# alexncoleman/WeaklySupervisedDL

Measured on AMD Instinct MI355X. Metric: SegmentationModel train img/s at B=16 256x256, higher is better.
Workload: dtype f32

## Files before the change

### include/wsdl_hip.h

```cpp
#ifndef WSDL_HIP_H
#define WSDL_HIP_H

#include <stddef.h>
#include <stdint.h>

#ifdef __cplusplus
extern "C" {
#endif

typedef void* wsdl_stream_t;

enum {
    WSDL_OK = 0,
    WSDL_EINVAL = -1,
    WSDL_EHIP = -2,
    WSDL_EWORKSPACE = -3
};

const char* wsdl_last_error(void);
int wsdl_launch_trace(int on);
const char* wsdl_last_launches(void);
int wsdl_version(void);
const char* wsdl_target_arch(void);

int wsdl_set_option(const char* name, int value);

enum { WSDL_PROF_IGEMM_128x128_A = 0,
       WSDL_PROF_IGEMM_128x128_U = 1,
       WSDL_PROF_IGEMM_128x64_A = 2, WSDL_PROF_IGEMM_128x64_U = 3,
       WSDL_PROF_IGEMM_64x256_A = 4, WSDL_PROF_IGEMM_64x256_U = 5,
       WSDL_PROF_IGEMM_64x128_A = 6, WSDL_PROF_IGEMM_64x128_U = 7,
       WSDL_PROF_WGRAD_128x128 = 8,
       WSDL_PROF_WGRAD_64x128 = 9,
       WSDL_PROF_WGRAD_FAST_128x128 = 10,
       WSDL_PROF_PAIRWISE = 11, WSDL_PROF_LAYERCAM = 12,
       WSDL_PROF_SPLIT_128x128 = 13,
       WSDL_PROF_SPLIT_128x64 = 14, WSDL_PROF_SPLIT_64x256 = 15, WSDL_PROF_SPLIT_64x128 = 16,
       WSDL_PROF_WGRAD_SPLIT32 = 17,
       WSDL_PROF_SPLIT_256x128 = 18,
       WSDL_PROF_STEM = 19,
       WSDL_PROF_WGRAD_SPLIT16D = 20,
       WSDL_PROF_SPLIT_GROUP = 21,
       WSDL_PROF_SPLIT_MULTI = 22,
       WSDL_PROF_NCLASSES = 23 };
const char* wsdl_prof_class_name(int cls);
int wsdl_prof_enable(int on);
int wsdl_prof_collect(int cls, long long* launches, double* total_ms, double* total_work,
                      double* total_work_executed ,
                      double* total_bytes );
int wsdl_prof_reset(void);

int wsdl_range_enable(int on);
int wsdl_range_push(const char* name);
int wsdl_range_pop(void);


size_t wsdl_conv2d_weight_layout_bytes(int Cout, int Cin, int kh, int kw, int dgrad, int* is_plain);
int wsdl_conv2d_prep_weights(const float* w, void* wt_fwd, void* wt_dgrad,
                             int Cout, int Cin, int kh, int kw,
                             const float* w_amax ,
                             wsdl_stream_t stream);

int wsdl_conv2d_fwd(const float* x, const void* wt_fwd, float* y,
                    int B, int Cin, int H, int W, int Cout, int kh, int kw,
                    int stride, int pad, int dil,
                    const float* scale, const float* shift, const float* residual, int relu,
                    long long x_bs, long long y_bs, long long res_bs,
                    const float* x_amax ,
                    float* y_amax ,
                    void* ws, size_t ws_bytes, wsdl_stream_t stream);
typedef struct wsdl_prep_desc {
    const float* w;
    void* wt_fwd;
    void* wt_dgrad;
    const float* w_amax;
    int Cout, Cin, taps, grid_x;
    int block_begin, reserved;
} wsdl_prep_desc;
int wsdl_conv2d_prep_weights_multi(const wsdl_prep_desc* desc, int n, int total_blocks, wsdl_stream_t stream);

size_t wsdl_conv2d_igemm_workspace(int B, int Cin, int H, int W, int Cout, int kh, int kw,
                                   int stride, int pad, int dil, int dgrad);

int wsdl_conv2d_dgrad(const float* dy, const void* wt_dgrad, float* dx,
                      int B, int Cin, int H, int W, int Cout, int kh, int kw,
                      int stride, int pad, int dil, int accumulate, const uint8_t* acc_mask,
                      long long dy_bs, const float* dy_amax, void* ws, size_t ws_bytes, wsdl_stream_t stream);
int wsdl_conv2d_fwd_group_ok(int n, int B, int Cin, int H, int W, int Cout);
size_t wsdl_conv2d_fwd_group_workspace(int n, const int* k, const int* dil, int B, int Cin, int H, int W, int Cout);
int wsdl_conv2d_fwd_group(int n, const float* x, const void* const* wt_fwd, float* const* y, const int* k, const int* dil,
                          int B, int Cin, int H, int W, int Cout, long long x_bs, const long long* y_bs,
                          const float* x_amax, void* ws, size_t ws_bytes, wsdl_stream_t stream);
int wsdl_conv2d_dgrad_multi_ok(int n, int B, int Cin, int H, int W, int Cout);
int wsdl_conv2d_dgrad_multi(int n, const float* const* dy, const void* const* wt_dgrad, const float* const* dy_amax,
                            const int* k, const int* dil, const long long* dy_bs, float* dx, int B, int Cin, int H, int W,
                            int Cout, int accumulate, wsdl_stream_t stream);

// ... 218 lines not shown
```

### weaklysuperviseddl_amd/csrc/common.hip

```cpp
#include "common.h"

#include <dlfcn.h>

#include <algorithm>
#include <mutex>
#include <vector>

namespace wsdl {

static thread_local char g_err[512] = "";
Opt g_range_sentinel{0};

void set_error(const char* fmt, ...) {
    va_list ap;
    va_start(ap, fmt);
    vsnprintf(g_err, sizeof(g_err), fmt, ap);
    va_end(ap);
}

std::atomic<int> g_trace_launches{0};
static thread_local char g_trace[2048] = "";
static thread_local size_t g_trace_len = 0;
void trace_launch(const char* fmt, ...) {
    if (g_trace_len + 4 >= sizeof(g_trace)) return;
// ... 47 lines not shown
    } else {
        if (hipEventCreate(&r.start) != hipSuccess) return;
        if (hipEventCreate(&r.stop) != hipSuccess) return;
    }
    (void)hipEventRecord(r.start, s);
    g_prof[cls].push_back(r);
    slot = reinterpret_cast<void*>(g_prof[cls].size());
}

ProfScope::~ProfScope() {
    if (g_ranges_on) g_roctx_pop();
    if (!slot) return;
    std::lock_guard<std::mutex> lk(g_prof_mu);
    size_t idx = reinterpret_cast<size_t>(slot) - 1;
    if (idx < g_prof[cls].size()) (void)hipEventRecord(g_prof[cls][idx].stop, s);
}

}

extern "C" {

int wsdl_launch_trace(int on) {
    wsdl::g_trace_launches.store(on ? 1 : 0);
    wsdl::g_trace[0] = 0;
    wsdl::g_trace_len = 0;
    return WSDL_OK;
}

const char* wsdl_last_launches(void) {
    static thread_local char out[sizeof(wsdl::g_trace)];
    memcpy(out, wsdl::g_trace, sizeof(out));
    wsdl::g_trace[0] = 0;
    wsdl::g_trace_len = 0;
    return out;
}

const char* wsdl_last_error(void) { return wsdl::g_err; }
int wsdl_version(void) { return 200; }
const char* wsdl_target_arch(void) { return "gfx950"; }

const char* wsdl_prof_class_name(int cls) {
    static const char* names[WSDL_PROF_NCLASSES] = {
        "conv_igemm_fast_kernel<128, 128, 2, 16>", "conv_igemm_kernel<128, 128, 2, false>",
        "conv_igemm_fast_kernel<128, 64, 2, 32>", "conv_igemm_kernel<128, 64, 2, false>",
        "conv_igemm_fast_kernel<64, 256, 1, 16>", "conv_igemm_kernel<64, 256, 1, false>",
        "conv_igemm_fast_kernel<64, 128, 1, 32>", "conv_igemm_kernel<64, 128, 1, false>",
        "conv_wgrad_kernel<128, 128, 2>", "conv_wgrad_kernel<64, 128, 1>", "conv_wgrad_fast_kernel<128, 128, 2, 16>",
        "pairwise_kernel", "layercam_partial_kernel",
        "conv_igemm_split_kernel<128, 128, 2, 16, 256, AR>", "conv_igemm_split_kernel<128, 64, 2, 32, 256, AR>",
        "conv_igemm_split_kernel<64, 256, 1, 16, 256, AR>", "conv_igemm_split_kernel<64, 128, 1, 32, 256, AR>",
        "conv_wgrad_split16_kernel<128, 128, false>", "conv_igemm_split_kernel<256, 128, 4, BK, 512, AR, false, false>",
        "stem_conv7x7s2_kernel", "conv_wgrad_split16d_kernel<MODE, DYRAW>",
        "conv_igemm_split_group_kernel<256, 128, 4, 16, 512, AR, false>",
        "conv_igemm_split_kernel<256, 128, 4, 16, 512, AR, false, true>"};
    return cls >= 0 && cls < WSDL_PROF_NCLASSES ? names[cls] : "?";
}

int wsdl_range_enable(int on) {
    if (on && !wsdl::load_roctx()) {
        wsdl::set_error("range_enable: librocprofiler-sdk-roctx.so / libroctx64.so could not be loaded");
        return WSDL_EINVAL;
    }
    wsdl::g_ranges_on = on != 0;
    return WSDL_OK;
}
int wsdl_range_push(const char* name) {
    if (wsdl::g_ranges_on && name) wsdl::g_roctx_push(name);
    return WSDL_OK;
}
int wsdl_range_pop(void) {
    if (wsdl::g_ranges_on) wsdl::g_roctx_pop();
    return WSDL_OK;
}

int wsdl_prof_enable(int on) {
    std::lock_guard<std::mutex> lk(wsdl::g_prof_mu);
    wsdl::g_prof_on = on != 0;
    return WSDL_OK;
}

int wsdl_prof_reset(void) {
    std::lock_guard<std::mutex> lk(wsdl::g_prof_mu);
    for (auto& v : wsdl::g_prof) {
        for (auto& r : v) wsdl::g_free_events.emplace_back(r.start, r.stop);
        v.clear();
    }
    return WSDL_OK;
}

int wsdl_prof_collect(int cls, long long* launches, double* total_ms, double* total_work,
                      double* total_work_executed, double* total_bytes) {
    WSDL_REQUIRE(cls >= 0 && cls < WSDL_PROF_NCLASSES, "prof class %d out of range", cls);
    std::lock_guard<std::mutex> lk(wsdl::g_prof_mu);
    double ms = 0.0, work = 0.0, exe = 0.0, byt = 0.0;
    for (auto& r : wsdl::g_prof[cls]) {
        WSDL_HIP_CHECK(hipEventSynchronize(r.stop));
        float t = 0.f;
        WSDL_HIP_CHECK(hipEventElapsedTime(&t, r.start, r.stop));
        ms += t;
        work += r.work;
        exe += r.executed;
        byt += r.bytes;
    }
    if (launches) *launches = (long long)wsdl::g_prof[cls].size();
    if (total_ms) *total_ms = ms;
    if (total_work) *total_work = work;
    if (total_work_executed) *total_work_executed = exe;
// ... 6 lines not shown
```

### weaklysuperviseddl_amd/csrc/conv_igemm.hip

```cpp
#include "common.h"

#include <type_traits>
#include <algorithm>
#include <cstdint>
#include <mutex>

typedef float f32x16 __attribute__((ext_vector_type(16)));

namespace {

constexpr int kThreads = 256;

struct ConvSrc {
    const float* x;
    const float* wt;
    const float* x_amax;
    int KH, KW, bh, ch, K, Cin;
    long long x_bs;
    unsigned x_bytes;
};

struct ConvP {
    const float* x;
    const float* wt;
// ... 1602 lines not shown
    bool fast;
    wgrad_tile(Cout, Cin, &BM, &BN, &fast);
    long long tiles = (long long)wsdl::cdiv(Cout, BM) * wsdl::cdiv(N, BN);
    const int chunks = wsdl::cdiv(P, 32);
    const long long smax = std::max<long long>(1, std::min<long long>(256, chunks / 8));
    if (wgrad_chunk32(Cout, Cin, N)) {
        tiles = (long long)wsdl::cdiv(Cout, BM) * wsdl::cdiv(std::max(n_live, BN), BN);
        const long long slots = 2 * kNumCU;
        long long best_s = 1;
        double best = -1.0;
        for (long long c = 1; c <= smax && tiles * c <= 5 * slots / 2; ++c) {
            const long long blocks = tiles * c, rounds = (blocks + slots - 1) / slots;
            double eff = (double)blocks / (double)(rounds * slots);
            if (blocks < slots) eff *= 0.9;
            if (eff > best + 0.03) { best = eff; best_s = c; }
        }
        if (tap_balance < 0.7 && n_live > BN && best_s + 1 <= smax) ++best_s;
        return (int)best_s;
    }
    long long s0 = (g_wgrad_blocks + tiles - 1) / tiles;
    if (s0 > smax) s0 = smax;
    if (s0 < 1) s0 = 1;
    long long s = s0;
    double best = 0.0;
    for (long long c = std::max<long long>(1, s0 - 1); c <= std::min<long long>(smax, s0 + 3); ++c) {
        const long long blocks = tiles * c, rounds = (blocks + kNumCU - 1) / kNumCU;
        const double eff = (double)blocks / (double)(rounds * kNumCU);
        if (eff > best + 0.02) { best = eff; s = c; }
    }
    return (int)s;
}


__global__ void transpose_add_kernel(const float* __restrict__ t, float* __restrict__ dw, int Cout, int Cin,
                                     int accumulate) {
    __shared__ float tile[32][33];
    const int co0 = blockIdx.x * 32, ci0 = blockIdx.y * 32;
    for (int r = threadIdx.y; r < 32; r += 8) {
        const int ci = ci0 + r, co = co0 + threadIdx.x;
        tile[r][threadIdx.x] = (ci < Cin && co < Cout) ? t[(long long)ci * Cout + co] : 0.f;
    }
    __syncthreads();
    for (int r = threadIdx.y; r < 32; r += 8) {
        const int co = co0 + r, ci = ci0 + threadIdx.x;
        if (co < Cout && ci < Cin) {
            const long long o = (long long)co * Cin + ci;
            dw[o] = accumulate ? dw[o] + tile[threadIdx.x][r] : tile[threadIdx.x][r];
        }
    }
}

bool wgrad_role_swap(int Cin, int Cout, int kh, int kw, int stride, int pad) {
    return kh == 1 && kw == 1 && stride == 1 && pad == 0 && !wgrad_chunk32(Cout, Cin, Cin) && wgrad_chunk32(Cin, Cout, Cout);
}

enum { WGRAD_REDUCE_PLAIN = 0, WGRAD_REDUCE_TILED, WGRAD_REDUCE_VEC4, WGRAD_REDUCE_MANY, WGRAD_REDUCE_MANY16 };
struct WgradReduce {
    const float* slab;
    float* dw;
    unsigned long long live;
    int S, Cout, Cin, T;
    int accumulate, kind;
    int grid_x, nblocks;
};
int wgrad_reduce_one(const WgradReduce& d, hipStream_t s) {
    switch (d.kind) {
        case WGRAD_REDUCE_TILED:
            hipLaunchKernelGGL(wgrad_reduce_tiled_kernel, dim3(d.grid_x, d.Cout), dim3(256), 0, s, d.slab, d.dw, d.S, d.Cout, d.Cin, d.T,
                               d.accumulate, d.live);
            break;
        case WGRAD_REDUCE_VEC4:
            hipLaunchKernelGGL(wgrad_reduce_vec4_kernel, dim3(d.nblocks), dim3(256), 0, s, reinterpret_cast<const float4*>(d.slab),
                               reinterpret_cast<float4*>(d.dw), d.S, (long long)d.Cout * d.Cin * d.T / 4, d.accumulate);
            break;
        case WGRAD_REDUCE_MANY:
            hipLaunchKernelGGL(wgrad_reduce_many_kernel, dim3(d.nblocks), dim3(256), 0, s, d.slab, d.dw, d.S, d.Cout, d.Cin, d.T,
                               d.accumulate, d.live);
            break;
        case WGRAD_REDUCE_MANY16:
            hipLaunchKernelGGL(wgrad_reduce_many16_kernel, dim3(d.nblocks), dim3(256), 0, s, d.slab, d.dw, d.S, d.Cout, d.Cin, d.T,
                               d.accumulate, d.live);
            break;
        default:
            hipLaunchKernelGGL(wgrad_reduce_kernel, dim3(d.nblocks), dim3(256), 0, s, d.slab, d.dw, d.S, d.Cout, d.Cin, d.T, d.accumulate,
                               d.live);
            break;
    }
    WSDL_LAUNCH_CHECK();
    return WSDL_OK;
}

template <int BM, int BN, int WM>
int launch_wgrad_fast(const WgradP& p, hipStream_t s, int S) {
    dim3 grid(p.N / BN, p.Cout / BM, S);
    hipLaunchKernelGGL((conv_wgrad_fast_kernel<BM, BN, WM, 16>), grid, dim3(kThreads), 2 * (BM + BN) * 17 * sizeof(float), s, p);
    WSDL_LAUNCH_CHECK();
    return WSDL_OK;
}

}

extern "C" {

int wsdl_set_option(const char* name, int value) {
    WSDL_REQUIRE(name, "set_option: null name");
    static std::mutex mu;
// ... 494 lines not shown
static int stem_wgrad_grid(int B, int OH, int OW) {
    const long long tiles = (long long)B * wsdl::cdiv(OH, kSwTH) * wsdl::cdiv(OW, kStemTW);
    return (int)std::min<long long>(tiles, kSwMaxGrid);
}

static size_t wgrad_dys_bytes(int Cout, int Cin, int N, int P) {
    if (!wgrad_chunk32(Cout, Cin, N)) return 0;
    const size_t n = (size_t)wsdl::cdiv(P, 32) * Cout * w2row_bytes(g_conv_arith);
    return n < (1ull << 31) ? n : 0;
}

static int wgrad_bands(int Cout, int Cin, int OW, int W, int kw, int stride, int pad, int dil, Band* bands) {
    int BM, BN;
    bool fast;
    wgrad_tile(Cout, Cin, &BM, &BN, &fast);
    bands[0] = Band{0, OW};
    if (!fast || stride != 1) return 1;
    if (wgrad_chunk32(Cout, Cin, kw * kw * Cin)) return 1;
    return column_bands(OW, W, 1, dil, -pad, 1, kw, bands);
}

size_t wsdl_conv2d_wgrad_presplit_bytes(int B, int Cin, int H, int W, int Cout, int kh, int kw, int stride, int pad, int dil) {
    int OH, OW;
    if (check_geom(B, Cin, H, W, Cout, kh, kw, stride, pad, dil, &OH, &OW)) return 0;
    if (g_conv_arith != 1 && g_conv_arith != 2) return 0;
    if (wgrad_role_swap(Cin, Cout, kh, kw, stride, pad)) return 0;
    const int N = kh * kw * Cin, P = B * OH * OW;
    const size_t bytes = wgrad_dys_bytes(Cout, Cin, N, P);
    if (!bytes || P % 32 != 0) return 0;
    const long long xb = (long long)B * Cin * H * W * 4, dyb = (long long)B * Cout * OH * OW * 4;
    if (xb >= (1ll << 31) || dyb >= (1ll << 31)) return 0;
    bool taps_aligned = true;
    for (int kx = 0; kx < kw; ++kx) taps_aligned = taps_aligned && (((kx * dil - pad) & 3) == 0);
    const bool direct = g_wgrad_direct && taps_aligned && stride == 1 && OW % 32 == 0 && W % 4 == 0 && (H * W) % 4 == 0;
    const bool dyraw = direct && g_wgrad_dyraw && (N / 128 <= 10 || g_wgrad_dyraw == 2) && (OH * OW) % 4 == 0;
    return dyraw ? 0 : bytes;
}

size_t wsdl_conv2d_wgrad_workspace(int B, int Cin, int H, int W, int Cout, int kh, int kw, int stride,
                                   int pad, int dil) {
    int OH, OW;
    if (check_geom(B, Cin, H, W, Cout, kh, kw, stride, pad, dil, &OH, &OW)) return 0;
    if (wgrad_role_swap(Cin, Cout, kh, kw, stride, pad))
        return wsdl::align_up((size_t)Cout * Cin * sizeof(float), 256) +
               wsdl_conv2d_wgrad_workspace(B, Cout, OH, OW, Cin, 1, 1, 1, 0, 1);
    const int N = kh * kw * Cin;
    Band bands[8];
    const int nb = wgrad_bands(Cout, Cin, OW, W, kw, stride, pad, dil, bands);
    const int n_live = __builtin_popcountll(live_taps(H, W, OH, OW, kh, kw, stride, pad, dil)) * Cin;
    size_t slabs = (size_t)nb * wgrad_splits(Cout, Cin, N, B * OH * OW, n_live, wgrad_tap_balance(H, OH, kh, stride, pad, dil)) *
                   Cout * N * sizeof(float);
    if (stem_wgrad_eligible(B, Cin, H, W, Cout, kh, kw, stride, pad, dil))
        slabs = std::max(slabs, (size_t)stem_wgrad_grid(B, OH, OW) * Cout * N * sizeof(float));
    return wsdl::align_up(slabs, 256) + wsdl::align_up(wgrad_dys_bytes(Cout, Cin, N, B * OH * OW), 256) +
           (g_wgrad_chan_scale ? wsdl::align_up((size_t)(Cin + Cout) * sizeof(float), 256) : 0);
}

struct WgradExtra {
    const float* x_chan;
    const float* dy_chan;
    const void* dy_presplit;
};
static int wgrad_impl(const float* x, const float* dy, float* dw, int B, int Cin, int H, int W,
                      int Cout, int kh, int kw, int stride, int pad, int dil, int accumulate,
                      long long x_bs, long long dy_bs, const float* x_amax, const float* dy_amax, void* ws,
                      size_t ws_bytes, wsdl_stream_t stream, WgradExtra ex = WgradExtra{}) {
    WSDL_REQUIRE(x && dy && dw && ws, "conv2d_wgrad: null pointer");
    int OH, OW;
    if (int rc = check_geom(B, Cin, H, W, Cout, kh, kw, stride, pad, dil, &OH, &OW)) return rc;
    if (wgrad_role_swap(Cin, Cout, kh, kw, stride, pad)) {
        const size_t t_bytes = wsdl::align_up((size_t)Cout * Cin * sizeof(float), 256);
        WSDL_REQUIRE(ws_bytes > t_bytes, "conv2d_wgrad: workspace too small");
        float* dwt = static_cast<float*>(ws);
        if (int rc = wgrad_impl(dy, x, dwt, B, Cout, OH, OW, Cin, 1, 1, 1, 0, 1, 0,
                                dy_bs ? dy_bs : (long long)Cout * OH * OW, x_bs ? x_bs : (long long)Cin * H * W,
                                dy_amax, x_amax, static_cast<char*>(ws) + t_bytes, ws_bytes - t_bytes, stream,
                                WgradExtra{ex.dy_chan, ex.x_chan, nullptr}))
            return rc;
        WSDL_TRACE("role-swapped (dW^T) + transpose");
        hipLaunchKernelGGL(transpose_add_kernel, dim3(wsdl::cdiv(Cout, 32), wsdl::cdiv(Cin, 32)), dim3(32, 8), 0,
                           wsdl::as_stream(stream), dwt, dw, Cout, Cin, accumulate);
        WSDL_LAUNCH_CHECK();
        return WSDL_OK;
    }
    WgradP p{};
    p.x = x; p.dy = dy; p.slab = static_cast<float*>(ws);
    p.B = B; p.Cin = Cin; p.H = H; p.W = W; p.Cout = Cout; p.OH = OH; p.OW = OW; p.KH = kh; p.KW = kw;
    p.stride = stride; p.pad = pad; p.dil = dil;
    p.N = kh * kw * Cin; p.P = B * OH * OW;
    p.x_bs = x_bs ? x_bs : (long long)Cin * H * W;
    p.dy_bs = dy_bs ? dy_bs : (long long)Cout * OH * OW;
    p.x_amax = x_amax;
    if (stem_wgrad_eligible(B, Cin, H, W, Cout, kh, kw, stride, pad, dil) &&
        (long long)B * wsdl::cdiv(OH, kSwTH) * wsdl::cdiv(OW, kStemTW) < (1ll << 31)) {
        const int G = stem_wgrad_grid(B, OH, OW);
        const size_t need = (size_t)G * Cout * p.N * sizeof(float);
        if (ws_bytes < need) {
            wsdl::set_error("conv2d_wgrad: workspace %zu < %zu bytes", ws_bytes, need);
            return WSDL_EWORKSPACE;
        }
        hipStream_t s = wsdl::as_stream(stream);
        const int tiles_w = wsdl::cdiv(OW, kStemTW), tiles_h = wsdl::cdiv(OH, kSwTH);
        {
            const double flops = 2.0 * p.P * (double)Cout * p.N;
            wsdl::ProfScope prof(WSDL_PROF_WGRAD_64x128, s, flops, flops, 4.0 * ((double)B * Cin * H * W + (double)p.P * Cout + (double)G * Cout * p.N));
            WSDL_TRACE("stem_wgrad7x7s2 fp32 workgroups=%d slabs=%d", G, G);
            hipLaunchKernelGGL(stem_wgrad7x7s2_kernel, dim3(G), dim3(256), 0, s, p, tiles_w, tiles_h, B * tiles_w * tiles_h);
            WSDL_LAUNCH_CHECK();
        }
        WgradReduce rd{};
        rd.slab = p.slab; rd.dw = dw; rd.S = G; rd.Cout = Cout; rd.Cin = Cin; rd.T = kh * kw; rd.accumulate = accumulate;
        rd.live = ~0ull;
        const long long total = (long long)Cout * p.N;
        if (G >= 64) {
            rd.kind = WGRAD_REDUCE_MANY16;
            rd.nblocks = (int)((total + 15) / 16);
        } else if (G >= 16) {
            rd.kind = WGRAD_REDUCE_MANY;
            rd.nblocks = (int)((total + 63) / 64);
        } else {
            rd.kind = WGRAD_REDUCE_PLAIN;
            rd.nblocks = (int)std::min<long long>((total + 255) / 256, 4096);
        }
        WSDL_TRACE("wgrad_reduce slabs=%d", G);
        return wgrad_reduce_one(rd, s);
    }
    const unsigned long long live_all = live_taps(H, W, OH, OW, kh, kw, stride, pad, dil);
    const int S = wgrad_splits(Cout, Cin, p.N, p.P, __builtin_popcountll(live_all) * Cin, wgrad_tap_balance(H, OH, kh, stride, pad, dil));
    Band bands[8];
    const int nb = wgrad_bands(Cout, Cin, OW, W, kw, stride, pad, dil, bands);
    if (nb == 1) bands[0] = Band{0, OW};
    const int S_total = nb * S;
    p.ow0 = 0; p.own = OW; p.slab0 = 0; p.nb = 1; p.splits = S;
    const size_t need = (size_t)S_total * Cout * p.N * sizeof(float);
    if (ws_bytes < need) {
        wsdl::set_error("conv2d_wgrad: workspace %zu < %zu bytes", ws_bytes, need);
        return WSDL_EWORKSPACE;
    }
    const int chunks = wsdl::cdiv(p.P, 32);
    p.chunks_per_split = wsdl::cdiv(chunks, S);
    hipStream_t s = wsdl::as_stream(stream);
    const long long xb = ((long long)(B - 1) * p.x_bs + (long long)Cin * H * W) * 4;
    const long long dyb = ((long long)(B - 1) * p.dy_bs + (long long)Cout * OH * OW) * 4;
    int tBM, tBN;
    bool fast;
    wgrad_tile(Cout, Cin, &tBM, &tBN, &fast);
    if (fast && (xb >= (1ll << 31) || dyb >= (1ll << 31))) {
        const long long img = std::max((long long)Cin * H * W, (long long)Cout * OH * OW) * 4;
        const long long bs = std::max(p.x_bs, p.dy_bs) * 4;
        WSDL_REQUIRE(B > 1 && img < (1ll << 31), "conv2d_wgrad: a single image of 2 GiB or more is not supported");
        long long per = ((1ll << 31) - 4 - img) / bs + 1;
        if (per < 1) per = 1;
        for (int b0 = 0; b0 < B; b0 += (int)per) {
            const int nb_img = (int)std::min<long long>(per, B - b0);
            if (int rc = wgrad_impl(x + (long long)b0 * p.x_bs, dy + (long long)b0 * p.dy_bs, dw, nb_img, Cin, H, W,
                                    Cout, kh, kw, stride, pad, dil, (accumulate || b0 > 0) ? 1 : 0, p.x_bs, p.dy_bs,
                                    x_amax, dy_amax, ws, ws_bytes, stream, WgradExtra{ex.x_chan, ex.dy_chan, nullptr}))
                return rc;
        }
        return WSDL_OK;
    }
    unsigned long long live_mask = ~0ull;
    {
        const double flops = 2.0 * p.P * (double)Cout * p.N;
        double executed = flops;
        const size_t dys_bytes = fast ? wgrad_dys_bytes(Cout, Cin, p.N, p.P) : 0;
        const size_t dys_off = wsdl::align_up(need, 256);
        const bool chunk32 = dys_bytes && ws_bytes >= dys_off + dys_bytes;
        if (wsdl::prof_enabled() && fast) {
            executed = 0.0;
            for (int i = 0; i < nb; ++i)
                executed += flops * ((double)bands[i].own / OW) *
                            wgrad_executed_fraction(B * OH * bands[i].own, OH, bands[i].ow0, bands[i].own, H, W, kh, kw,
                                                    stride, pad, dil, chunk32 ? 32 : 16);
        }
        bool taps_aligned = true;
        for (int kx = 0; kx < kw; ++kx) taps_aligned = taps_aligned && (((kx * dil - pad) & 3) == 0);
        const bool direct = chunk32 && g_conv_arith && g_wgrad_direct && taps_aligned &&
// ... 215 lines not shown
```

### weaklysuperviseddl_amd/csrc/conv_split.h

```cpp
#pragma once

typedef __bf16 bf16x8 __attribute__((ext_vector_type(8)));
typedef __bf16 bf16x2 __attribute__((ext_vector_type(2)));
typedef _Float16 half8 __attribute__((ext_vector_type(8)));
typedef float f32x4 __attribute__((ext_vector_type(4)));

__device__ __forceinline__ void split3(float x0, float x1, unsigned& h, unsigned& m, unsigned& l) {
    f32x2 v = {x0, x1};
    h = __builtin_bit_cast(unsigned, __builtin_convertvector(v, bf16x2));
    f32x2 r = {x0 - __builtin_bit_cast(float, h << 16), x1 - __builtin_bit_cast(float, h & 0xffff0000u)};
    m = __builtin_bit_cast(unsigned, __builtin_convertvector(r, bf16x2));
    f32x2 s = {r[0] - __builtin_bit_cast(float, m << 16), r[1] - __builtin_bit_cast(float, m & 0xffff0000u)};
    l = __builtin_bit_cast(unsigned, __builtin_convertvector(s, bf16x2));
}

__device__ __forceinline__ void split2hs(float x0, float x1, unsigned& h, unsigned& l) {
    f32x2 v = {x0, x1};
    const half2v hv = __builtin_convertvector(v, half2v);
    h = __builtin_bit_cast(unsigned, hv);
    f32x2 r = {(x0 - (float)hv[0]) * 2048.f, (x1 - (float)hv[1]) * 2048.f};
    l = __builtin_bit_cast(unsigned, __builtin_convertvector(r, half2v));
}

template <int AR> struct SplitArith;
// ... 1356 lines not shown
#pragma unroll
            for (int i = 0; i < TMI; ++i) {
                const half8 a0 = *reinterpret_cast<const half8*>(Ab + i * 16 * ROW + fr0);
                const half8 a1 = *reinterpret_cast<const half8*>(Ab + i * 16 * ROW + fr1);
#pragma unroll
                for (int j = 0; j < TNI; ++j) {
                    f32x4 c = acc[i][j];
                    c = __builtin_amdgcn_mfma_f32_16x16x32_f16(a1, b[j][0], c, 0, 0, 0);
                    c = __builtin_amdgcn_mfma_f32_16x16x32_f16(a0, b[j][1], c, 0, 0, 0);
                    c = __builtin_amdgcn_mfma_f32_16x16x32_f16(a0, b[j][0], c, 0, 0, 0);
                    acc[i][j] = c;
                }
            }
            if (c1 < chunk_end) store_a(std::integral_constant<int, 1 - S>{}, buf ^ 1);
            buf ^= 1;
            c0 = c1;
            c1 = c2;
        };
        while (c0 < chunk_end) {
            step(S0{});
            if (c0 >= chunk_end) break;
            step(S1{});
        }
    };
    static_assert(MODE == 0, "only the aligned loop is instantiated (the misaligned-tap loops were removed in round 4)");
    run(std::integral_constant<int, 0>{});

    float* slab = p.slab + (long long)(p.slab0 + bz) * p.Cout * p.N;
    if constexpr (CS) {
#pragma unroll
        for (int i = 0; i < TMI; ++i)
#pragma unroll
            for (int r = 0; r < 4; ++r) {
                const int row = i * 16 + lg * 4 + r, co = m0 + row;
                const int edr = edy_s[row];
#pragma unroll
                for (int j = 0; j < TNI; ++j)
                    slab[(long long)co * p.N + n0 + wid * 32 + j * 16 + l15] = ldexpf(acc[i][j][r], -(exr[j] + edr));
            }
        return;
    }
#pragma unroll
    for (int i = 0; i < TMI; ++i)
#pragma unroll
        for (int j = 0; j < TNI; ++j) {
            const int n = n0 + wid * 32 + j * 16 + l15;
#pragma unroll
            for (int r = 0; r < 4; ++r) {
                const int co = m0 + i * 16 + lg * 4 + r;
                slab[(long long)co * p.N + n] = acc[i][j][r] * out_scale;
            }
        }
}
```

### weaklysuperviseddl_amd/ops.py

```python
import ctypes as C

import os

import threading

import numpy as np
import torch

from ._lib import lib, check, WsdlError

_vp = C.c_void_p


_raw_stream = torch._C._cuda_getCurrentRawStream
_cur_device = torch._C._cuda_getDevice


def raw_stream(device=None):
    idx = device.index if (device is not None and device.index is not None) else _cur_device()
    return _raw_stream(idx)


def _stream():
    return _raw_stream(_cur_device())
# ... 609 lines not shown
    if any(ws[0] != Cout or ws[1] != Cin for ws in wshapes):
        raise WsdlError("conv2d_fwd_group: the problems must share their channel counts")
    IA, PA, LA = C.c_int * n, _vp * n, C.c_longlong * n
    ks, ds = IA(*[int(ws[2]) for ws in wshapes]), IA(*[int(d) for d in dils])
    nws = lib().wsdl_conv2d_fwd_group_workspace(n, ks, ds, B, Cin, H, W, Cout)
    if nws == 0:
        raise WsdlError("conv2d_fwd_group: geometry not supported")
    ws = workspace(nws, x.device)
    if outs is None:
        outs = [torch.empty(B, Cout, H, W, device=x.device, dtype=torch.float32) for _ in range(n)]
    bss = []
    dense = []
    for o in outs:
        t, bs = _planes(o, "out")
        if t is not o:
            raise WsdlError("conv2d_fwd_group: preallocated outputs must be dense planes")
        dense.append(t)
        bss.append(bs)
    check(lib().wsdl_conv2d_fwd_group(n, _p(x), PA(*[_p(w) for w in wfs]), PA(*[_p(t) for t in dense]), ks, ds, B, Cin, H, W,
                                      Cout, x_bs, LA(*bss), _p(x_amax), _p(ws), ws.numel(), _stream()))
    return outs


def dgrad_multi_ok(n, xshape, cout):
    B, Cin, H, W = xshape
    return bool(lib().wsdl_conv2d_dgrad_multi_ok(int(n), B, Cin, H, W, int(cout)))


def conv2d_dgrad_multi(dys, wds, wshapes, dils, xshape, accumulate_into=None, dy_amaxes=None):
    n = len(dys)
    B, Cin, H, W = xshape
    Cout = wshapes[0][0]
    amaxes = []
    dense = []
    bss = []
    for i in range(n):
        if wshapes[i][0] != Cout or wshapes[i][1] != Cin:
            raise WsdlError("conv2d_dgrad_multi: the sources must share their channel counts")
        a = dy_amaxes[i] if dy_amaxes is not None and dy_amaxes[i] is not None else \
            amax_of(dys[i], _split_kc(Cout, wshapes[i][2] * wshapes[i][3]))
        t, bs = _planes(dys[i], "dy")
        amaxes.append(a)
        dense.append(t)
        bss.append(bs)
    dx = accumulate_into if accumulate_into is not None else torch.empty(xshape, device=dys[0].device, dtype=torch.float32)
    PA, IA, LA = _vp * n, C.c_int * n, C.c_longlong * n
    check(lib().wsdl_conv2d_dgrad_multi(n, PA(*[_p(t) for t in dense]), PA(*[_p(w) for w in wds]), PA(*[_p(a) for a in amaxes]),
                                        IA(*[int(ws[2]) for ws in wshapes]), IA(*[int(d) for d in dils]), LA(*bss), _p(dx),
                                        B, Cin, H, W, Cout, int(accumulate_into is not None), _stream()))
    dx._wsdl_fresh = True
    return dx


def _wgrad_split(wshape):
    return CONV_ARITH[0] == 1 and wshape[0] % 128 == 0 and wshape[1] % 128 == 0


def wgrad_presplit_bytes(xshape, wshape, stride, pad, dil):
    B, Cin, H, W = xshape
    Cout, _, kh, kw = wshape
    return _ws_bytes("wsdl_conv2d_wgrad_presplit_bytes", B, Cin, H, W, Cout, kh, kw, stride, pad, dil)


def conv2d_wgrad(x, dy, wshape, stride, pad, dil, out=None, accumulate=False, x_amax=None, dy_amax=None, stream=None,
                 x_camax=None, dy_camax=None, dy_presplit=None):
    if dy_camax is None:
        dy_presplit = None
    elif dy_presplit is None:
        dy_camax_p = getattr(dy, "_wsdl_camax", None)
        if dy_camax_p is dy_camax:
            dy_presplit = getattr(dy, "_wsdl_presplit", None)
    if stream is not None and stream != _stream():
        split = _wgrad_split(wshape)
        if out is None or (split and (x_amax is None or dy_amax is None)):
            raise WsdlError("conv2d_wgrad(stream=): pass out, x_amax and dy_amax (resolved on the current stream)")
        if _planes(x, "x")[0] is not x or _planes(dy, "dy")[0] is not dy:
            raise WsdlError("conv2d_wgrad(stream=): operands must already be dense planes")
    if x_amax is None:
        x_amax = amax_of(x, _wgrad_split(wshape))
    if dy_amax is None:
        dy_amax = amax_of(dy, _wgrad_split(wshape))
    x, x_bs = _planes(x, "x")
    dy, dy_bs = _planes(dy, "dy")
    B, Cin, H, W = x.shape
    Cout, _, kh, kw = wshape
    geom = (B, Cin, H, W, Cout, kh, kw, stride, pad, dil)
    nbytes = _ws_bytes("wsdl_conv2d_wgrad_workspace", *geom)
    if nbytes == 0:
        raise WsdlError("conv2d_wgrad: bad geometry " + repr(geom))
    ws = workspace(nbytes, x.device, stream)
    if out is None:
        out = torch.empty(wshape, device=x.device, dtype=torch.float32)
        accumulate = False
    check(lib().wsdl_conv2d_wgrad_ex(_p(x), _p(dy), _p(out), *geom, int(accumulate), x_bs, dy_bs, _p(x_amax), _p(dy_amax),
                                     _p(x_camax), _p(dy_camax), _p(dy_presplit), _p(ws), ws.numel(),
                                     _stream() if stream is None else stream))
    return out


def bias_grad(dy, out=None, accumulate=False):
    dy, dy_bs = _planes(dy, "dy")
    B, Cc, H, W = dy.shape
    if out is None:
        out = torch.empty(Cc, device=dy.device, dtype=torch.float32)
        accumulate = False
    check(lib().wsdl_bias_grad(_p(dy), _p(out), B, Cc, H * W, dy_bs, int(accumulate), _stream()))
    return out


def bn_fold(bn_weight, bn_bias, running_mean, running_var, eps):
    Cc = bn_weight.numel()
    scale = torch.empty(Cc, device=bn_weight.device, dtype=torch.float32)
    shift = torch.empty_like(scale)
    check(lib().wsdl_bn_fold(_p(_dense(bn_weight)), _p(_dense(bn_bias)), _p(_dense(running_mean)),
                             _p(_dense(running_var)), float(eps), _p(scale), _p(shift), Cc, _stream()))
    return scale, shift


def bn_fold_bias(bn_weight, bn_bias, running_mean, running_var, conv_bias, eps):
    Cc = bn_weight.numel()
    scale = torch.empty(Cc, device=bn_weight.device, dtype=torch.float32)
    shift = torch.empty_like(scale)
    check(lib().wsdl_bn_fold_bias(_p(_dense(bn_weight)), _p(_dense(bn_bias)), _p(_dense(running_mean)),
                                  _p(_dense(running_var)), _p(_dense(conv_bias)), float(eps), _p(scale), _p(shift), Cc,
                                  _stream()))
    return scale, shift


CHAN_AMAX = [os.environ.get("WSDL_CHAN_AMAX", "1") != "0"]
DY_PRESPLIT = [os.environ.get("WSDL_DY_PRESPLIT", "1") != "0"]


def _bn_resident(B, Cc, HW, backward):
    key = ("wsdl_bn_channel_resident", (B, Cc, HW, backward))
# ... 76 lines not shown
    if dx_amax is not None:
        _publish_amax(dx, dx_amax)
    if camax is not None:
        dx._wsdl_camax = camax
        if presplit is not None:
            dx._wsdl_presplit = presplit
    dx._wsdl_fresh = True
    if dres is not None:
        dres._wsdl_fresh = True
    return dx, dgamma, dbeta, dres


def _owned(t):
    return (t is not None and getattr(t, "_wsdl_fresh", False) and t._base is None and t.is_contiguous()
            and t.dtype == torch.float32 and not t.requires_grad)


def affine_act_bwd(dy, y, scale, relu, want_dconv=True, want_dres=False):
    dy = _dense(dy, "dy")
    B, Cc, H, W = dy.shape
    dconv = torch.empty_like(dy) if want_dconv else None
    dres = torch.empty_like(dy) if want_dres else None
    amax = amax_slot(dy.device) if (want_dconv and CONV_ARITH[0] == 1) else None
    check(lib().wsdl_affine_act_bwd(_p(dy), _p(_dense(y) if relu else None), _p(scale), _p(dconv), _p(dres), B, Cc,
                                    H * W, int(relu), _p(amax), _stream()))
    if amax is not None:
        _publish_amax(dconv, amax)
    return dconv, dres


OVERLAP_WGRAD = [True]
WGRAD_AFTER_DGRAD = [False]
LAST_WGRAD_ON_MAIN = [os.environ.get("WSDL_LAST_WGRAD_ON_MAIN", "1") != "0"]
_side_streams = {}


def side_stream(device):
    if device.index is None:
        device = _norm_device(device)
    st = _side_streams.get(device)
    if st is None:
        st = _side_streams[device] = torch.cuda.Stream(device=device)
    return st


def join_side_stream(device):
    st = _side_streams.get(_norm_device(device))
    if st is not None:
        stream_wait(raw_stream(device), st)


def _wgrad_into(param, x, dconv, wshape, stride, pad, dil, sink, x_amax=None, last=False, x_camax=None):
    accumulate = not sink.take_fresh(param)
    split = _wgrad_split(wshape)
    x_amax = x_amax if x_amax is not None else amax_of(x, split)
    dy_amax = amax_of(dconv, split)
    dy_camax = getattr(dconv, "_wsdl_camax", None) if split else None
    dy_presplit = getattr(dconv, "_wsdl_presplit", None) if dy_camax is not None else None
    if not split:
        x_camax = None
    elif x_camax is None:
        x_camax = getattr(x, "_wsdl_camax", None)
    if x_camax is not None and x_camax.numel() != wshape[1]:
        x_camax = None
    if OVERLAP_WGRAD[0] and not (last and LAST_WGRAD_ON_MAIN[0]):
        x, dconv = _planes(x, "x")[0], _planes(dconv, "dy")[0]
        side = side_stream(x.device)
        hside = side.cuda_stream
        stream_wait(hside, _stream())
        conv2d_wgrad(x, dconv, wshape, stride, pad, dil, out=param.grad, accumulate=accumulate, x_amax=x_amax,
                     dy_amax=dy_amax, stream=hside, x_camax=x_camax, dy_camax=dy_camax,
                     dy_presplit=dy_presplit)
        for t in (x_camax, dy_camax, dy_presplit):
            if t is not None:
                t.record_stream(side)
        x.record_stream(side)
        dconv.record_stream(side)
    else:
        conv2d_wgrad(x, dconv, wshape, stride, pad, dil, out=param.grad, accumulate=accumulate, x_amax=x_amax,
                     dy_amax=dy_amax, x_camax=x_camax, dy_camax=dy_camax, dy_presplit=dy_presplit)
    sink.grad_ready(param)


def _sink_of(param):
    sink = getattr(param, "_wsdl_grad_sink", None)
    if sink is None or param.grad is None or not param.grad.is_cuda:
        return None
    return sink


def _alias(t):
    return torch.empty(0, device=t.device, dtype=t.dtype).set_(t.untyped_storage(), t.storage_offset(), t.shape, t.stride())


class IdentityLink:
    __slots__ = ("pending", "projection")

    def __init__(self, projection=False):
        self.pending = None
        self.projection = projection


IDENTITY_LINK = [os.environ.get("WSDL_IDENTITY_LINK", "1") != "0"]


class _ConvBNAct(torch.autograd.Function):

    @staticmethod
    def forward(ctx, x, weight, gamma, beta, residual, running_mean, running_var, stride, pad, dil, relu,
                momentum, eps, cache=None, passthrough=False, link=None, out_holder=None):
        ctx.link = link
        if link is not None:
            ctx.set_materialize_grads(False)
        wf, wd = _cached_prep(cache, weight, x.requires_grad)
        x_amax = amax_of(x, _split_kc(x.shape[1], weight.shape[2] * weight.shape[3]) or _wgrad_split(weight.shape))
        conv = conv2d_fwd(x, wf, weight.shape, stride, pad, dil, x_amax=x_amax)
        y, mean, invstd, rbits = bn_train_fwd(conv, _dense(gamma), _dense(beta), running_mean, running_var, momentum, eps,
                                              residual, relu, out=_alias(out_holder[0]) if out_holder else None,
                                              want_mask=True, mask_if=bool(relu) and residual is not None,
                                              amax_into=out_holder[1] if out_holder else None)
        ctx.cfg = (stride, pad, dil, relu, tuple(weight.shape), tuple(x.shape), residual is not None)
        ctx.params = (weight, gamma, beta)
        ctx.x_amax = x_amax
        ctx.x_camax = getattr(x, "_wsdl_camax", None)
        ctx.save_for_backward(x, conv, y if (relu and residual is not None and rbits is None) else None, gamma, mean, invstd,
                              wd, beta if relu else None, rbits)
        if passthrough:
            xv = x.view_as(x)
            if x_amax is not None:
                _publish_amax(xv, x_amax)
            if ctx.x_camax is not None:
                xv._wsdl_camax = ctx.x_camax
            return y, xv
        return y

    @staticmethod
    def backward(ctx, dy, dxres=None):
        x, conv, y, gamma, mean, invstd, wd, beta_s, rbits = ctx.saved_tensors
        stride, pad, dil, relu, wshape, xshape, has_res = ctx.cfg
        pw, pg, pb = ctx.params
        need_res = has_res and ctx.needs_input_grad[4]
        link = ctx.link
        if dy is None:
            raise WsdlError("conv -> BatchNorm node: no gradient arrived for its output")
        alias_dres = False
        if (link is not None and need_res and rbits is not None and IDENTITY_LINK[0] and tuple(dy.shape) == tuple(conv.shape)
                and dy.is_contiguous()):
            if link.projection:
                link.pending = (dy, rbits)
                need_res, alias_dres = False, True
            elif _owned(dy):
                link.pending = (dy, rbits)
                need_res = False
        shortcut_bits = None
        if link is not None and link.projection and not has_res:
            if link.pending is not None:
                src, shortcut_bits = link.pending
                link.pending = None
                if src.data_ptr() != dy.data_ptr() or tuple(src.shape) != tuple(dy.shape):
                    raise WsdlError("projection shortcut: the gradient that arrived is not the block output's (autograd "
                                    "copied or summed it) - set WSDL_IDENTITY_LINK=0")
        if shortcut_bits is not None:
            relu_b, y_b, beta_b, bits_b = True, None, None, shortcut_bits
        else:
            relu_b, y_b, beta_b, bits_b = relu, y, beta_s, rbits
        sg = _sink_of(pg) if (ctx.needs_input_grad[2] and ctx.needs_input_grad[3] and _sink_of(pg) is _sink_of(pb)) else None
        psb = wgrad_presplit_bytes(xshape, wshape, stride, pad, dil) if (ctx.needs_input_grad[1] and _sink_of(pw) is not None) else 0
        if sg is not None:
# ... 1336 lines not shown


def add_scalars(a, b):
    return _AddAct.apply(a.reshape(1), b.reshape(1), False).reshape(())


def kl_div_batchmean(xn, s):
    return _KLDivBatchMean.apply(xn, s)


RANGES = [False]


def ranges_enable(on=True):
    check(lib().wsdl_range_enable(int(bool(on))))
    RANGES[0] = bool(on)


class prof_range:
    __slots__ = ("name",)

    def __init__(self, name):
        self.name = name

    def __enter__(self):
        if RANGES[0]:
            lib().wsdl_range_push(self.name.encode())

    def __exit__(self, *exc):
        if RANGES[0]:
            lib().wsdl_range_pop()
        return False


if os.environ.get("WSDL_ROCTX") == "1":
    try:
        ranges_enable(True)
    except Exception:
        RANGES[0] = False


PROF_ON = [False]


def prof_enable(on):
    check(lib().wsdl_prof_enable(int(on)))
    PROF_ON[0] = bool(on)


def prof_reset():
    check(lib().wsdl_prof_reset())


PROF_NCLASSES = 23


def prof_class_name(cls):
    return lib().wsdl_prof_class_name(int(cls)).decode()


def prof_collect(cls):
    n, ms, work, exe, byt = C.c_longlong(0), C.c_double(0), C.c_double(0), C.c_double(0), C.c_double(0)
    check(lib().wsdl_prof_collect(int(cls), C.byref(n), C.byref(ms), C.byref(work), C.byref(exe), C.byref(byt)))
    return n.value, ms.value, work.value, exe.value, byt.value
```

Baseline: 916.9.

## Add whole-dW split-fp16 wgrad kernel for small 64-channel convolutions

```diff
diff --git a/include/wsdl_hip.h b/include/wsdl_hip.h
--- a/include/wsdl_hip.h
+++ b/include/wsdl_hip.h
@@ -42,7 +42,8 @@
        WSDL_PROF_WGRAD_SPLIT16D = 20,
        WSDL_PROF_SPLIT_GROUP = 21,
        WSDL_PROF_SPLIT_MULTI = 22,
-       WSDL_PROF_NCLASSES = 23 };
+       WSDL_PROF_WGRAD_WHOLE16 = 23,
+       WSDL_PROF_NCLASSES = 24 };
 const char* wsdl_prof_class_name(int cls);
 int wsdl_prof_enable(int on);
 int wsdl_prof_collect(int cls, long long* launches, double* total_ms, double* total_work,
diff --git a/weaklysuperviseddl_amd/csrc/common.hip b/weaklysuperviseddl_amd/csrc/common.hip
--- a/weaklysuperviseddl_amd/csrc/common.hip
+++ b/weaklysuperviseddl_amd/csrc/common.hip
@@ -123,7 +123,8 @@
         "conv_wgrad_split16_kernel<128, 128, false>", "conv_igemm_split_kernel<256, 128, 4, BK, 512, AR, false, false>",
         "stem_conv7x7s2_kernel", "conv_wgrad_split16d_kernel<MODE, DYRAW>",
         "conv_igemm_split_group_kernel<256, 128, 4, 16, 512, AR, false>",
-        "conv_igemm_split_kernel<256, 128, 4, 16, 512, AR, false, true>"};
+        "conv_igemm_split_kernel<256, 128, 4, 16, 512, AR, false, true>",
+        "conv_wgrad_split_whole16_kernel<CO, CI, T>"};
     return cls >= 0 && cls < WSDL_PROF_NCLASSES ? names[cls] : "?";
 }
 
diff --git a/weaklysuperviseddl_amd/csrc/conv_igemm.hip b/weaklysuperviseddl_amd/csrc/conv_igemm.hip
--- a/weaklysuperviseddl_amd/csrc/conv_igemm.hip
+++ b/weaklysuperviseddl_amd/csrc/conv_igemm.hip
@@ -1678,6 +1678,19 @@
 
 bool wgrad_role_swap(int Cin, int Cout, int kh, int kw, int stride, int pad) {
     return kh == 1 && kw == 1 && stride == 1 && pad == 0 && !wgrad_chunk32(Cout, Cin, Cin) && wgrad_chunk32(Cin, Cout, Cout);
+}
+
+bool wgrad_whole16(int Cout, int Cin, int kh, int kw, int stride, int dil) {
+    if (!g_wgrad_split || g_conv_arith < 1 || stride != 1 || dil != 1 || kh != kw || (kh != 1 && kh != 3)) return false;
+    auto ch = [](int c) { return c == 64 || c == 128 || c == 256; };
+    return ch(Cout) && ch(Cin) && (Cout == 64 || Cin == 64) && Cout * Cin * kh * kw <= 36864;
+}
+int wgrad_whole16_groups(int Cout, int Cin, int T, int P, int* cps) {
+    const int chunks = wsdl::cdiv(P, 32);
+    const int target = 256;
+    const int per = wsdl::cdiv(chunks, std::min(target, chunks));
+    if (cps) *cps = per;
+    return wsdl::cdiv(chunks, per);
 }
 
 enum { WGRAD_REDUCE_PLAIN = 0, WGRAD_REDUCE_TILED, WGRAD_REDUCE_VEC4, WGRAD_REDUCE_MANY, WGRAD_REDUCE_MANY16 };
@@ -2278,6 +2291,8 @@
                    Cout * N * sizeof(float);
     if (stem_wgrad_eligible(B, Cin, H, W, Cout, kh, kw, stride, pad, dil))
         slabs = std::max(slabs, (size_t)stem_wgrad_grid(B, OH, OW) * Cout * N * sizeof(float));
+    if (wgrad_whole16(Cout, Cin, kh, kw, stride, dil))
+        slabs = std::max(slabs, (size_t)wgrad_whole16_groups(Cout, Cin, kh * kw, B * OH * OW, nullptr) * Cout * N * sizeof(float));
     return wsdl::align_up(slabs, 256) + wsdl::align_up(wgrad_dys_bytes(Cout, Cin, N, B * OH * OW), 256) +
            (g_wgrad_chan_scale ? wsdl::align_up((size_t)(Cin + Cout) * sizeof(float), 256) : 0);
 }
@@ -2350,6 +2365,64 @@
         }
         WSDL_TRACE("wgrad_reduce slabs=%d", G);
         return wgrad_reduce_one(rd, s);
+    }
+    if (wgrad_whole16(Cout, Cin, kh, kw, stride, dil) && x_amax && dy_amax) {
+        const long long xb = ((long long)(B - 1) * p.x_bs + (long long)Cin * H * W) * 4;
+        const long long dyb = ((long long)(B - 1) * p.dy_bs + (long long)Cout * OH * OW) * 4;
+        if (xb < (1ll << 31) && dyb < (1ll << 31)) {
+            const int T = kh * kw;
+            const int G = wgrad_whole16_groups(Cout, Cin, T, p.P, &p.chunks_per_split);
+            const size_t need = (size_t)G * Cout * p.N * sizeof(float);
+            if (ws_bytes < need) {
+                wsdl::set_error("conv2d_wgrad: workspace %zu < %zu bytes", ws_bytes, need);
+                return WSDL_EWORKSPACE;
+            }
+            hipStream_t s = wsdl::as_stream(stream);
+            p.x_bytes = (unsigned)xb;
+            p.dy_bytes = (unsigned)dyb;
+            p.xa_stride = p.da_stride = 0;
+            if (ex.x_chan) { p.x_amax = ex.x_chan; p.xa_stride = 1; }
+            if (ex.dy_chan) { dy_amax = ex.dy_chan; p.da_stride = 1; }
+            {
+                const double flops = 2.0 * p.P * (double)Cout * p.N;
+                wsdl::ProfScope prof(WSDL_PROF_WGRAD_WHOLE16, s, flops, flops,
+                                     4.0 * ((double)B * Cin * H * W + (double)p.P * Cout + (double)G * Cout * p.N));
+                WSDL_TRACE("wgrad_whole16<%d,%d> G=%d taps=%d cs=%d grid=%dx%d", Cout, Cin, G, T,
+                           (int)(p.xa_stride || p.da_stride), G, p.chunks_per_split);
+#define WSDL_WHOLE16(CO, CI, TT)                                                                                          \
+    if (Cout == CO && Cin == CI && T == TT)                                                                               \
+        hipLaunchKernelGGL((conv_wgrad_split_whole16_kernel<CO, CI, TT>), dim3(G), dim3(kThreads), 0, s, p, dy_amax)
+                WSDL_WHOLE16(64, 64, 9);
+                else WSDL_WHOLE16(64, 64, 1);
+                else WSDL_WHOLE16(256, 64, 1);
+                else WSDL_WHOLE16(64, 256, 1);
+                else WSDL_WHOLE16(128, 64, 1);
+                else WSDL_WHOLE16(64, 128, 1);
+                else WSDL_REQUIRE(false, "conv2d_wgrad: no whole-dW kernel for %d x %d x %d", Cout, Cin, T);
+#undef WSDL_WHOLE16
+                WSDL_LAUNCH_CHECK();
+            }
+            WgradReduce rd{};
+            rd.slab = p.slab; rd.dw = dw; rd.S = G; rd.Cout = Cout; rd.Cin = Cin; rd.T = T; rd.accumulate = accumulate;
+            rd.live = ~0ull;
+            const long long total = (long long)Cout * p.N;
+            if (G >= 64) {
+                rd.kind = WGRAD_REDUCE_MANY16;
+                rd.nblocks = (int)((total + 15) / 16);
+            } else if (T > 1) {
+                rd.kind = WGRAD_REDUCE_TILED;
+                rd.grid_x = wsdl::cdiv(Cin, 32);
+                rd.nblocks = rd.grid_x * Cout;
+            } else if ((reinterpret_cast<uintptr_t>(dw) & 15) == 0) {
+                rd.kind = WGRAD_REDUCE_VEC4;
+                rd.nblocks = (int)std::min<long long>((total / 4 + 255) / 256, 8192);
+            } else {
+                rd.kind = WGRAD_REDUCE_PLAIN;
+                rd.nblocks = (int)std::min<long long>((total + 255) / 256, 4096);
+            }
+            WSDL_TRACE("wgrad_reduce slabs=%d", G);
+            return wgrad_reduce_one(rd, s);
+        }
     }
     const unsigned long long live_all = live_taps(H, W, OH, OW, kh, kw, stride, pad, dil);
     const int S = wgrad_splits(Cout, Cin, p.N, p.P, __builtin_popcountll(live_all) * Cin, wgrad_tap_balance(H, OH, kh, stride, pad, dil));
diff --git a/weaklysuperviseddl_amd/csrc/conv_split.h b/weaklysuperviseddl_amd/csrc/conv_split.h
--- a/weaklysuperviseddl_amd/csrc/conv_split.h
+++ b/weaklysuperviseddl_amd/csrc/conv_split.h
@@ -1432,3 +1432,185 @@
             }
         }
 }
+
+template <int I, int N, typename F>
+__device__ __forceinline__ void whole16_for(F&& f) {
+    if constexpr (I < N) {
+        f(std::integral_constant<int, I>{});
+        whole16_for<I + 1, N>(f);
+    }
+}
+
+template <int R>
+__device__ __forceinline__ void whole16_load(unsigned (&rb)[R / 8], const __amdgpu_buffer_rsrc_t rs, unsigned voff, int plane) {
+#pragma unroll
+    for (int e = 0; e < R / 8; ++e)
+        rb[e] = __builtin_amdgcn_raw_buffer_load_b32(rs, voff, (unsigned)(((e & 1) + 16 * (e >> 1)) * plane) * 4u, 0);
+}
+template <int R>
+__device__ __forceinline__ void whole16_store(unsigned char* tile, const unsigned (&rb)[R / 8], const float* sc, bool even,
+                                              unsigned st_row, unsigned st_u0, unsigned st_u1) {
+#pragma unroll
+    for (int i = 0; i < R / 16; ++i) {
+        const unsigned give = even ? rb[2 * i + 1] : rb[2 * i];
+        const unsigned recv = (unsigned)__builtin_amdgcn_mov_dpp((int)give, 0xB1, 0xF, 0xF, true);
+        const unsigned x0 = even ? rb[2 * i] : recv;
+        const unsigned x1 = even ? recv : rb[2 * i + 1];
+        unsigned ph, pl;
+        const float s = sc[16 * i];
+        split2h(__builtin_bit_cast(float, x0) * s, __builtin_bit_cast(float, x1) * s, ph, pl);
+        unsigned char* d = tile + st_row + i * 16 * kW16Row;
+        *reinterpret_cast<unsigned*>(d + st_u0) = ph;
+        *reinterpret_cast<unsigned*>(d + st_u1) = pl;
+    }
+}
+
+template <int CO, int CI, int T>
+__global__ __launch_bounds__(kThreads, (T == 1 && CO + CI <= 192) ? 2 : 1) void conv_wgrad_split_whole16_kernel(WgradP p, const float* __restrict__ dy_amax) {
+    static_assert(T == 1 || T == 9, "1x1 or 3x3");
+    static_assert(CO % 64 == 0 && CI % 64 == 0 && CO * CI * T <= 36864, "all of dW in 144 accumulator registers");
+    constexpr int ROW = kW16Row, KW = T == 9 ? 3 : 1;
+    constexpr bool WIDE_M = CO >= CI;
+    constexpr int TMI = WIDE_M ? CO / 64 : CO / 16, TNI = WIDE_M ? CI / 16 : CI / 64;
+    constexpr int DS = T == 1 ? 2 : 1;
+    constexpr unsigned kOOB = 0x80000000u;
+
+    __shared__ __attribute__((aligned(16))) unsigned char As[2][CO * ROW];
+    __shared__ __attribute__((aligned(16))) unsigned char Bs[2][CI * ROW];
+    __shared__ float xsc_s[CI], dsc_s[CO];
+    __shared__ int xe_s[CI], de_s[CO];
+
+    const int tid = threadIdx.x;
+    const int lane = tid & 63, wid = tid >> 6;
+    const int px = tid & 31, hw = tid >> 5;
+    const int OHOW = p.OH * p.OW, HW = p.H * p.W;
+    const __amdgpu_buffer_rsrc_t rx =
+        __builtin_amdgcn_make_buffer_rsrc(const_cast<float*>(p.x), 0, (int)p.x_bytes, 0x00020000);
+    const __amdgpu_buffer_rsrc_t rdy =
+        __builtin_amdgcn_make_buffer_rsrc(const_cast<float*>(p.dy), 0, (int)p.dy_bytes, 0x00020000);
+    for (int i = tid; i < CI; i += kThreads) {
+        int e_;
+        xsc_s[i] = pow2_scale(p.x_amax[i * p.xa_stride], e_);
+        xe_s[i] = e_;
+    }
+    for (int i = tid; i < CO; i += kThreads) {
+        int e_;
+        dsc_s[i] = pow2_scale(dy_amax[i * p.da_stride], e_);
+        de_s[i] = e_;
+    }
+    __syncthreads();
+    const float* xsr = xsc_s + 2 * hw + (px & 1);
+    const float* dsr = dsc_s + 2 * hw + (px & 1);
+
+    const int chunk_begin = blockIdx.x * p.chunks_per_split;
+    const int chunk_end = min(chunk_begin + p.chunks_per_split, (p.P + 31) / 32);
+
+    bool d_ok = false;
+    int d_oh = 0, d_ow = 0;
+    unsigned d_x = 0;
+    auto decode = [&](int c) {
+        const int pix = c * 32 + px;
+        d_ok = c < chunk_end && pix < p.P;
+        const int b = pix / OHOW, rr = pix - b * OHOW;
+        d_oh = rr / p.OW;
+        d_ow = rr - d_oh * p.OW;
+        d_x = (unsigned)((long long)b * p.x_bs) + (unsigned)(2 * hw * HW);
+    };
+    auto x_off = [&](int t) {
+        const int ih = d_oh + t / KW - p.pad, iw = d_ow + t % KW - p.pad;
+        return (d_ok && ih >= 0 && ih < p.H && iw >= 0 && iw < p.W) ? (d_x + (unsigned)(ih * p.W + iw)) * 4u : kOOB;
+    };
+    auto dy_off = [&](int c) {
+        const int pix = c * 32 + px;
+        if (c >= chunk_end || pix >= p.P) return kOOB;
+        const int b = pix / OHOW, rr = pix - b * OHOW;
+        return ((unsigned)((long long)b * p.dy_bs) + (unsigned)(rr + 2 * hw * OHOW)) * 4u;
+    };
+
+    f32x4 acc[T][TMI][TNI];
+#pragma unroll
+    for (int t = 0; t < T; ++t)
+#pragma unroll
+        for (int i = 0; i < TMI; ++i)
+#pragma unroll
+            for (int j = 0; j < TNI; ++j) acc[t][i][j] = f32x4{0.f, 0.f, 0.f, 0.f};
+
+    unsigned rbx[2][CI / 8], rbd[DS][CO / 8];
+    const bool even = (px & 1) == 0;
+    const int pair = px >> 1;
+    const unsigned st_row = (unsigned)((2 * hw + (even ? 0 : 1)) * ROW + (pair & 3) * 4);
+    const unsigned st_u0 = (unsigned)(((pair >> 2) ^ (hw & 7)) << 4), st_u1 = (unsigned)(((4 + (pair >> 2)) ^ (hw & 7)) << 4);
+    const int l15 = lane & 15, lg = lane >> 4;
+    const unsigned fr0 = (unsigned)(l15 * ROW + ((lg ^ (l15 >> 1)) << 4)), fr1 = (unsigned)(l15 * ROW + (((4 + lg) ^ (l15 >> 1)) << 4));
+    const int row0 = WIDE_M ? wid * (CO / 4) : 0, col0 = WIDE_M ? 0 : wid * (CI / 4);
+
+    half8 a[TMI][2];
+    auto step = [&](auto par_c, auto t_c, int c) {
+        constexpr int PAR = decltype(par_c)::value, t = decltype(t_c)::value;
+        constexpr int XS = (PAR * T + t) & 1, DSL = T == 1 ? PAR : 0;
+        whole16_store<CI>(Bs[XS], rbx[XS], xsr, even, st_row, st_u0, st_u1);
+        if constexpr (t == 0) whole16_store<CO>(As[PAR], rbd[DSL], dsr, even, st_row, st_u0, st_u1);
+        constexpr int tn = (t + 2) % T;
+        if constexpr (tn == 0) decode(c + (t + 2) / T);
+        whole16_load<CI>(rbx[XS], rx, x_off(tn), HW);
+        if constexpr (t == 0) whole16_load<CO>(rbd[DSL], rdy, dy_off(c + DS), OHOW);
+        lds_barrier();
+        if constexpr (t == 0) {
+            const unsigned char* Ab = As[PAR] + row0 * ROW;
+#pragma unroll
+            for (int i = 0; i < TMI; ++i) {
+                a[i][0] = *reinterpret_cast<const half8*>(Ab + i * 16 * ROW + fr0);
+                a[i][1] = *reinterpret_cast<const half8*>(Ab + i * 16 * ROW + fr1);
+            }
+        }
+        const unsigned char* Bb = Bs[XS] + col0 * ROW;
+#pragma unroll
+        for (int j = 0; j < TNI; ++j) {
+            const half8 b0 = *reinterpret_cast<const half8*>(Bb + j * 16 * ROW + fr0);
+            const half8 b1 = *reinterpret_cast<const half8*>(Bb + j * 16 * ROW + fr1);
+#pragma unroll
+            for (int i = 0; i < TMI; ++i) {
+                f32x4 cc = acc[t][i][j];
+                cc = __builtin_amdgcn_mfma_f32_16x16x32_f16(a[i][1], b0, cc, 0, 0, 0);
+                cc = __builtin_amdgcn_mfma_f32_16x16x32_f16(a[i][0], b1, cc, 0, 0, 0);
+                cc = __builtin_amdgcn_mfma_f32_16x16x32_f16(a[i][0], b0, cc, 0, 0, 0);
+                acc[t][i][j] = cc;
+            }
+        }
+    };
+    using P0 = std::integral_constant<int, 0>;
+    using P1 = std::integral_constant<int, 1>;
+
+    decode(chunk_begin);
+    whole16_load<CI>(rbx[0], rx, x_off(0), HW);
+    whole16_load<CO>(rbd[0], rdy, dy_off(chunk_begin), OHOW);
+    if constexpr (T == 1) {
+        decode(chunk_begin + 1);
+        whole16_load<CI>(rbx[1], rx, x_off(0), HW);
+        whole16_load<CO>(rbd[DS - 1], rdy, dy_off(chunk_begin + 1), OHOW);
+    } else {
+        whole16_load<CI>(rbx[1], rx, x_off(1), HW);
+    }
+    for (int c = chunk_begin; c < chunk_end; c += 2) {
+        whole16_for<0, T>([&](auto t_c) { step(P0{}, t_c, c); });
+        if (c + 1 >= chunk_end) break;
+        whole16_for<0, T>([&](auto t_c) { step(P1{}, t_c, c + 1); });
+    }
+
+    float* slab = p.slab + (long long)blockIdx.x * CO * p.N;
+    int en[TNI];
+#pragma unroll
+    for (int j = 0; j < TNI; ++j) en[j] = xe_s[col0 + j * 16 + l15];
+#pragma unroll
+    for (int i = 0; i < TMI; ++i)
+#pragma unroll
+        for (int r = 0; r < 4; ++r) {
+            const int co = row0 + i * 16 + lg * 4 + r;
+            const int edr = de_s[co];
+#pragma unroll
+            for (int t = 0; t < T; ++t)
+#pragma unroll
+                for (int j = 0; j < TNI; ++j)
+                    slab[(long long)co * p.N + t * CI + col0 + j * 16 + l15] = ldexpf(acc[t][i][j][r], -(en[j] + edr));
+        }
+}
diff --git a/weaklysuperviseddl_amd/ops.py b/weaklysuperviseddl_amd/ops.py
--- a/weaklysuperviseddl_amd/ops.py
+++ b/weaklysuperviseddl_amd/ops.py
@@ -685,8 +685,14 @@
     return dx
 
 
-def _wgrad_split(wshape):
-    return CONV_ARITH[0] == 1 and wshape[0] % 128 == 0 and wshape[1] % 128 == 0
+def _wgrad_split(wshape, stride=1, dil=1):
+    if CONV_ARITH[0] != 1:
+        return False
+    co, ci, kh, kw = (int(v) for v in wshape)
+    if co % 128 == 0 and ci % 128 == 0:
+        return True
+    return (stride == 1 and dil == 1 and kh == kw and kh in (1, 3) and co in (64, 128, 256) and ci in (64, 128, 256)
+            and 64 in (co, ci) and co * ci * kh * kw <= 36864)
 
 
 def wgrad_presplit_bytes(xshape, wshape, stride, pad, dil):
@@ -704,15 +710,15 @@
         if dy_camax_p is dy_camax:
             dy_presplit = getattr(dy, "_wsdl_presplit", None)
     if stream is not None and stream != _stream():
-        split = _wgrad_split(wshape)
+        split = _wgrad_split(wshape, stride, dil)
         if out is None or (split and (x_amax is None or dy_amax is None)):
             raise WsdlError("conv2d_wgrad(stream=): pass out, x_amax and dy_amax (resolved on the current stream)")
         if _planes(x, "x")[0] is not x or _planes(dy, "dy")[0] is not dy:
             raise WsdlError("conv2d_wgrad(stream=): operands must already be dense planes")
     if x_amax is None:
-        x_amax = amax_of(x, _wgrad_split(wshape))
+        x_amax = amax_of(x, _wgrad_split(wshape, stride, dil))
     if dy_amax is None:
-        dy_amax = amax_of(dy, _wgrad_split(wshape))
+        dy_amax = amax_of(dy, _wgrad_split(wshape, stride, dil))
     x, x_bs = _planes(x, "x")
     dy, dy_bs = _planes(dy, "dy")
     B, Cin, H, W = x.shape
@@ -895,7 +901,7 @@
 
 def _wgrad_into(param, x, dconv, wshape, stride, pad, dil, sink, x_amax=None, last=False, x_camax=None):
     accumulate = not sink.take_fresh(param)
-    split = _wgrad_split(wshape)
+    split = _wgrad_split(wshape, stride, dil)
     x_amax = x_amax if x_amax is not None else amax_of(x, split)
     dy_amax = amax_of(dconv, split)
     dy_camax = getattr(dconv, "_wsdl_camax", None) if split else None
@@ -956,7 +962,7 @@
         if link is not None:
             ctx.set_materialize_grads(False)
         wf, wd = _cached_prep(cache, weight, x.requires_grad)
-        x_amax = amax_of(x, _split_kc(x.shape[1], weight.shape[2] * weight.shape[3]) or _wgrad_split(weight.shape))
+        x_amax = amax_of(x, _split_kc(x.shape[1], weight.shape[2] * weight.shape[3]) or _wgrad_split(weight.shape, stride, dil))
         conv = conv2d_fwd(x, wf, weight.shape, stride, pad, dil, x_amax=x_amax)
         y, mean, invstd, rbits = bn_train_fwd(conv, _dense(gamma), _dense(beta), running_mean, running_var, momentum, eps,
                                               residual, relu, out=_alias(out_holder[0]) if out_holder else None,
@@ -2399,7 +2405,7 @@
     check(lib().wsdl_prof_reset())
 
 
-PROF_NCLASSES = 23
+PROF_NCLASSES = 24
 
 
 def prof_class_name(cls):
```

Result: no change. 915.8 (-0.1%).
